# spartan-array/spartan

Measured on AMD Instinct MI355X. Metric: spartan.dot TFLOP/s (+ map/reduce HBM GB/s), higher is better.
Workload: dtype f32

## Files before the change

### spartan_amd/csrc/gemm_split.hpp

```cpp
#pragma once

typedef __bf16 gs_bf16x8 __attribute__((ext_vector_type(8)));
typedef __bf16 gs_bf16x4 __attribute__((ext_vector_type(4)));

namespace {

constexpr int GS_BK = 16;
constexpr int GS_RB = GS_BK * 2;
constexpr int GS_WN = 4;
constexpr unsigned GS_WIN_LO = (127u - 40u) << 23;
constexpr unsigned GS_WIN_HI = (127u + 40u) << 23;
constexpr size_t GS_IMAGE_CAP = (size_t)2 << 30;
constexpr size_t GS_WS_HEAD = 512;

template <int WN>
struct GsCfg {
  static constexpr int BM = 256, BN = 64 * WN, NW = 2 * WN, THREADS = 64 * NW;
  static constexpr int A_BYTES = BM * GS_RB, B_BYTES = BN * GS_RB;
  static constexpr int STAGE_BYTES = 3 * A_BYTES + 3 * B_BYTES;
  static constexpr int SMEM_BYTES = 2 * STAGE_BYTES;
  static constexpr int APW = A_BYTES / 1024 / NW, BPW = B_BYTES / 1024 / NW;
  static constexpr int NPIECES = 3 * APW + 3 * BPW;
  static constexpr int SLOTS = SP_CUS * (WN == 4 ? 1 : 2);
  static_assert(APW >= 1 && BPW >= 1 && APW * NW * 1024 == A_BYTES && BPW * NW * 1024 == B_BYTES, "tile / waves mismatch");
  static_assert(NPIECES * 4 <= 48, "one piece after every fourth MFMA");
};

__device__ __forceinline__ bool gs_outside(float v) {
  const unsigned b = __float_as_uint(v) & 0x7fffffffu;
  return b != 0u && (b < GS_WIN_LO || b >= GS_WIN_HI);
}

__device__ __forceinline__ void gs_cut(float v, __bf16& h, __bf16& m, __bf16& l) {
  h = (__bf16)v;
  const float r1 = v - (float)h;
  m = (__bf16)r1;
  l = (__bf16)(r1 - (float)m);
}

__device__ __forceinline__ void gs_raise(bool bad, unsigned* flag) {
  if (__any(bad) && (threadIdx.x & 63) == 0) atomicOr(flag, 1u);
}

__global__ __launch_bounds__(256) void sp_gemm_cut_rows_kernel(const float* __restrict__ A, int64_t lda, int M, int K,
                                                               __bf16* __restrict__ Ah, int64_t img,
                                                               unsigned* __restrict__ flag) {
  const int q = threadIdx.x & 7, row = blockIdx.x * 32 + (threadIdx.x >> 3);
  const int kpad = (K + GS_BK - 1) / GS_BK * GS_BK;
  bool bad = false;
  if (row < M) {
    const float* __restrict__ a = A + (int64_t)row * lda;
#pragma unroll
    for (int it = 0; it < 8; ++it) {
      const int k = blockIdx.y * 256 + it * 32 + 4 * q;
      if (k >= kpad) break;
      f32x4 v = {0.f, 0.f, 0.f, 0.f};
      if (k + 4 <= K) {
        v = *(const f32x4*)(a + k);
      } else {
#pragma unroll
        for (int e = 0; e < 4; ++e)
          if (k + e < K) v[e] = a[k + e];
      }
      gs_bf16x4 h, m, l;
#pragma unroll
      for (int e = 0; e < 4; ++e) {
        bad |= gs_outside(v[e]);
        __bf16 hh, mm, ll;
        gs_cut(v[e], hh, mm, ll);
        h[e] = hh;
        m[e] = mm;
        l[e] = ll;
      }
      const int64_t at = ((int64_t)(k >> 4) * M + row) * GS_BK + (k & 15);
      *(gs_bf16x4*)(Ah + at) = h;
      *(gs_bf16x4*)(Ah + img + at) = m;
      *(gs_bf16x4*)(Ah + 2 * img + at) = l;
    }
  }
  gs_raise(bad, flag);
}

__global__ __launch_bounds__(256) void sp_gemm_cut_cols_kernel(const float* __restrict__ B, int64_t ldb, int N, int K,
                                                               __bf16* __restrict__ Bh, int64_t img,
                                                               unsigned* __restrict__ flag) {
  __shared__ __attribute__((aligned(16))) __bf16 s[3][256 * GS_BK];
  const int n0 = blockIdx.x * 256, col = n0 + threadIdx.x, k0 = blockIdx.y * GS_BK;
  float v[GS_BK];
#pragma unroll
  for (int e = 0; e < GS_BK; ++e) v[e] = (col < N && k0 + e < K) ? B[(int64_t)(k0 + e) * ldb + col] : 0.f;
  bool bad = false;
  gs_bf16x8 h[2], m[2], l[2];
#pragma unroll
  for (int e = 0; e < GS_BK; ++e) {
    bad |= gs_outside(v[e]);
    __bf16 hh, mm, ll;
    gs_cut(v[e], hh, mm, ll);
    h[e >> 3][e & 7] = hh;
    m[e >> 3][e & 7] = mm;
    l[e >> 3][e & 7] = ll;
  }
#pragma unroll
  for (int c = 0; c < 2; ++c) {
    *(gs_bf16x8*)(&s[0][threadIdx.x * GS_BK + 8 * c]) = h[c];
    *(gs_bf16x8*)(&s[1][threadIdx.x * GS_BK + 8 * c]) = m[c];
    *(gs_bf16x8*)(&s[2][threadIdx.x * GS_BK + 8 * c]) = l[c];
  }
  __syncthreads();
  const int64_t base = ((int64_t)blockIdx.y * N + n0) * GS_BK;
#pragma unroll
  for (int p = 0; p < 3; ++p)
#pragma unroll
    for (int c = 0; c < 2; ++c) {
      const int at = (c * 256 + threadIdx.x) * 8;
      if (n0 + at / GS_BK < N) *(gs_bf16x8*)(Bh + p * img + base + at) = *(const gs_bf16x8*)(&s[p][at]);
    }
  gs_raise(bad, flag);
}

template <int WN>
__global__ __launch_bounds__(GsCfg<WN>::THREADS, 2) void sp_gemm_glds_kernel_bf16x3(
    const char* __restrict__ Ah, int64_t a_img, const char* __restrict__ Bh, int64_t b_img, float* __restrict__ C,
    int64_t ldc, int M, int N, int KT, int accumulate, int tiles_m, int tiles_n, const unsigned* __restrict__ flag) {
  using G = GsCfg<WN>;
  constexpr int APW = G::APW, BPW = G::BPW, NPIECES = G::NPIECES;
  extern __shared__ __attribute__((aligned(16))) char gs_smem[];
  if (*flag != 0u) return;
  int tm, tn;
  sp_gemm_tile_of_block(blockIdx.x, gridDim.x, tiles_m, tiles_n, tm, tn);
  const int m0 = tm * G::BM, n0 = tn * G::BN;
  const int tid = threadIdx.x, lane = tid & 63;
  const int wid = __builtin_amdgcn_readfirstlane(tid >> 6);
  const int wm = wid / WN, wn = wid % WN;
  const int l31 = lane & 31, lh = lane >> 5;

  unsigned a_off[APW], b_off[BPW];
#pragma unroll
  for (int j = 0; j < APW; ++j) {
    const int slot = (wid * APW + j) * 64 + lane;
    int row = slot >> 1;
    const int q = (slot & 1) ^ ((row >> 4) & 1);
    if (m0 + row > M - 1) row = M - 1 - m0;
    a_off[j] = (unsigned)(row * GS_RB + q * 16);
  }
#pragma unroll
  for (int j = 0; j < BPW; ++j) {
    const int slot = (wid * BPW + j) * 64 + lane;
    int row = slot >> 1;
    const int q = (slot & 1) ^ ((row >> 4) & 1);
    if (n0 + row > N - 1) row = N - 1 - n0;
    b_off[j] = (unsigned)(row * GS_RB + q * 16);
  }
  const char* __restrict__ Ablk = Ah + (int64_t)m0 * GS_RB;
  const char* __restrict__ Bblk = Bh + (int64_t)n0 * GS_RB;
  const int64_t a_slab = (int64_t)M * GS_RB, b_slab = (int64_t)N * GS_RB;
  const unsigned s_base = SP_LDS_ADDR(gs_smem);

#define GS_PIECE(i)                                                                                    \
  do {                                                                                                 \
    if ((i) < 3 * APW) {                                                                               \
      const int p_ = (i) / APW, j_ = (i) % APW;                                                        \
      SP_GLDS_S(Ablk + p_ * a_img + ka_, a_off[j_], st_ + p_ * G::A_BYTES + (wid * APW + j_) * 1024);  \
    } else {                                                                                           \
      const int p_ = ((i) - 3 * APW) / BPW, j_ = ((i) - 3 * APW) % BPW;                                \
      SP_GLDS_S(Bblk + p_ * b_img + kb_, b_off[j_],                                                    \
                st_ + 3 * G::A_BYTES + p_ * G::B_BYTES + (wid * BPW + j_) * 1024);                     \
    }                                                                                                  \
  } while (0)

  f32x16 acc[4][2];
#pragma unroll
  for (int i = 0; i < 4; ++i)
#pragma unroll
    for (int j = 0; j < 2; ++j)
#pragma unroll
      for (int r = 0; r < 16; ++r) acc[i][j][r] = 0.f;

  {
    const int64_t ka_ = 0, kb_ = 0;
    const unsigned st_ = s_base;
#pragma unroll
    for (int i = 0; i < NPIECES; ++i) GS_PIECE(i);
  }
  SP_GLDS_LANDED();
  __syncthreads();

  const int fslot = (lh ^ ((l31 >> 4) & 1)) * 16;
  const int a_frag = (wm * 128 + l31) * GS_RB + fslot;
  const int b_frag = 3 * G::A_BYTES + (wn * 64 + l31) * GS_RB + fslot;

  for (int t = 0; t < KT; ++t) {
    const bool more = t + 1 < KT;
    const int64_t ka_ = (int64_t)(t + 1) * a_slab, kb_ = (int64_t)(t + 1) * b_slab;
    const unsigned st_ = s_base + (unsigned)((t + 1) & 1) * G::STAGE_BYTES;
    const char* st = gs_smem + (t & 1) * G::STAGE_BYTES;
    gs_bf16x8 af[3][4], bf[3][2];
#pragma unroll
    for (int p = 0; p < 3; ++p) {
#pragma unroll
      for (int i = 0; i < 4; ++i) af[p][i] = *(const gs_bf16x8*)(st + p * G::A_BYTES + a_frag + i * 32 * GS_RB);
#pragma unroll
      for (int j = 0; j < 2; ++j) bf[p][j] = *(const gs_bf16x8*)(st + p * G::B_BYTES + b_frag + j * 32 * GS_RB);
    }
    int piece = 0;
#pragma unroll
    for (int idx = 0; idx < 48; ++idx) {
      const int term = idx >> 3, i = (idx & 7) >> 1, j = idx & 1;
      const int pa = term == 0 ? 2 : (term == 2 || term == 3) ? 1 : 0;
      const int pb = term == 1 ? 2 : (term == 2 || term == 4) ? 1 : 0;
      acc[i][j] = __builtin_amdgcn_mfma_f32_32x32x16_bf16(af[pa][i], bf[pb][j], acc[i][j], 0, 0, 0);
      if (idx % 4 == 3 && piece < NPIECES) {
        __builtin_amdgcn_sched_barrier(0);
        if (more) GS_PIECE(piece);
        __builtin_amdgcn_sched_barrier(0);
        ++piece;
      }
    }
    if (more) SP_GLDS_LANDED();
    __syncthreads();
  }
#undef GS_PIECE

#pragma unroll
  for (int i = 0; i < 4; ++i) {
#pragma unroll
    for (int j = 0; j < 2; ++j) {
      const int col = n0 + wn * 64 + j * 32 + l31;
#pragma unroll
      for (int r = 0; r < 16; ++r) {
        const int row = m0 + wm * 128 + i * 32 + (r & 3) + 8 * (r >> 2) + 4 * lh;
        if (row < M && col < N) {
          float* p = C + (int64_t)row * ldc + col;
          float v = acc[i][j][r];
          if (accumulate) v += *p;
          *p = v;
        }
      }
    }
  }
}

template <typename Cfg, int BM, int BN, int WM, int WN, int WGS>
__global__ __launch_bounds__(Cfg::THREADS, WGS) void sp_gemm_f32_gated_kernel(
    const float* __restrict__ A, int64_t lda, const float* __restrict__ B, int64_t ldb, float* __restrict__ C,
    int64_t ldc, int M, int N, int K, int accumulate, int tiles_m, int tiles_n, const unsigned* __restrict__ flag) {
  if (*flag == 0u) return;
  sp_gemm_glds_body<Cfg, BM, BN, WM, WN>(A, lda, B, ldb, C, ldc, M, N, K, accumulate, tiles_m, tiles_n);
}

#define GS_CUT_BYTES_PER_S 3.0e12
#define GS_ISSUED_FLOPS 1.1e15
static bool sp_gemm_bf16_plan(int64_t M, int64_t N, int64_t K) {
  static int mode = -2;
  if (mode == -2) {
    const char* e = getenv("SP_GEMM_SPLIT");
    mode = e ? atoi(e) : 1;
  }
  using G = GsCfg<GS_WN>;
  if (mode == 0 || K < 16 || N % 4 != 0 || N < 4 || M < 1 || M > 2147483647LL || N > 2147483647LL || K > 2147483647LL)
    return false;
  const int64_t tb = ((M + 255) / 256) * ((N + 127) / 128);
  if (tb < 2 * SP_CUS || tb >= 2147483647LL) return false;
  double dp_cost;
  if (sp_gemm_dp_choice(M, N, &dp_cost) != 6 || sp_sk_plan(M, N, K)) return false;
  const int64_t KT = (K + GS_BK - 1) / GS_BK;
  if ((double)KT * 3.0 * GS_RB * ((double)M + (double)N) > (double)GS_IMAGE_CAP) return false;
  const double fp32_s = dp_cost * 128.0 * 128.0 * (double)K * 2.0 / (157.3e12 * 0.95 / SP_CUS);
  const int64_t tiles = ((M + G::BM - 1) / G::BM) * ((N + G::BN - 1) / G::BN);
  const int64_t rounds = (tiles + G::SLOTS - 1) / G::SLOTS;
  const double main_s = (double)rounds * G::SLOTS * (6.0 * 2.0 * G::BM * G::BN * (double)K) / GS_ISSUED_FLOPS;
  const double cut_s = 10.0 * ((double)M + (double)N) * (double)K / GS_CUT_BYTES_PER_S;
  return (main_s + cut_s + 20e-6) < 0.92 * fp32_s;
}

static size_t sp_gemm_bf16_ws_bytes(int64_t M, int64_t N, int64_t K) {
  return GS_WS_HEAD + (size_t)((K + GS_BK - 1) / GS_BK) * 3 * GS_RB * (size_t)(M + N);
}

static int sp_gemm_bf16_launch(const float* A, int64_t lda, const float* B, int64_t ldb, float* C, int64_t ldc, int64_t M,
                               int64_t N, int64_t K, int acc, void* ws, hipStream_t st) {
  using G = GsCfg<GS_WN>;
  char* base = (char*)(((uintptr_t)ws + 255) & ~(uintptr_t)255);
  unsigned* flag = (unsigned*)base;
  const int64_t KT = (K + GS_BK - 1) / GS_BK;
  const int64_t a_img = KT * M * GS_RB, b_img = KT * N * GS_RB;
  char* Aimg = base + 256;
  char* Bimg = Aimg + 3 * a_img;
  const int64_t tiles_m = (M + G::BM - 1) / G::BM, tiles_n = (N + G::BN - 1) / G::BN;
  auto kern = sp_gemm_glds_kernel_bf16x3<GS_WN>;
  using FCfg = GldsCfg<256, 128, 2, 2>;
  auto gated = sp_gemm_f32_gated_kernel<FCfg, 256, 128, 2, 2, 2>;
  static bool attr_set = false;
  if (!attr_set) {
    SP_HIP(hipFuncSetAttribute((const void*)kern, hipFuncAttributeMaxDynamicSharedMemorySize, G::SMEM_BYTES));
    SP_HIP(hipFuncSetAttribute((const void*)gated, hipFuncAttributeMaxDynamicSharedMemorySize, FCfg::LDS_BYTES));
    attr_set = true;
  }
  SP_HIP(hipMemsetAsync(flag, 0, 256, st));
  hipLaunchKernelGGL(sp_gemm_cut_rows_kernel, dim3((unsigned)((M + 31) / 32), (unsigned)((K + 255) / 256)), dim3(256), 0, st,
                     A, lda, (int)M, (int)K, (__bf16*)Aimg, a_img / 2, flag);
  hipLaunchKernelGGL(sp_gemm_cut_cols_kernel, dim3((unsigned)((N + 255) / 256), (unsigned)KT), dim3(256), 0, st, B, ldb,
                     (int)N, (int)K, (__bf16*)Bimg, b_img / 2, flag);
  hipLaunchKernelGGL(kern, dim3((unsigned)(tiles_m * tiles_n)), dim3(G::THREADS), G::SMEM_BYTES, st, (const char*)Aimg,
                     a_img, (const char*)Bimg, b_img, C, ldc, (int)M, (int)N, (int)KT, acc, (int)tiles_m, (int)tiles_n,
                     (const unsigned*)flag);
  const int64_t ftm = (M + 255) / 256, ftn = (N + 127) / 128;
  hipLaunchKernelGGL(gated, dim3((unsigned)(ftm * ftn)), dim3(FCfg::THREADS), FCfg::LDS_BYTES, st, A, lda, B, ldb, C, ldc,
                     (int)M, (int)N, (int)K, acc, (int)ftm, (int)ftn, (const unsigned*)flag);
  SP_CHECK_LAUNCH();
  return 0;
}

}
```

### spartan_amd/csrc/sp_common.hpp

```cpp
#pragma once
#include <hip/hip_runtime.h>
#include <stdint.h>
#ifndef __HIPCC_RTC__
#include <stdio.h>
#include <string.h>
#endif

#include "../../include/spartan_hip.h"

void sp_set_error(const char* fmt, ...);

#define SP_FAIL(...)          \
  do {                        \
    sp_set_error(__VA_ARGS__); \
    return 1;                 \
  } while (0)

#define SP_HIP(expr)                                                              \
  do {                                                                            \
    hipError_t e_ = (expr);                                                       \
    if (e_ != hipSuccess) {                                                       \
      sp_set_error("%s:%d: %s failed: %s", __FILE__, __LINE__, #expr,             \
                   hipGetErrorString(e_));                                        \
      return 1;                                                                   \
    }                                                                             \
  } while (0)

#define SP_CHECK_LAUNCH()                                                         \
  do {                                                                            \
    hipError_t e_ = hipGetLastError();                                            \
    if (e_ != hipSuccess) {                                                       \
      sp_set_error("%s:%d: kernel launch failed: %s", __FILE__, __LINE__,         \
                   hipGetErrorString(e_));                                        \
      return 1;                                                                   \
    }                                                                             \
  } while (0)

__host__ __device__ static inline size_t sp_dtype_size(int32_t dt) {
  switch (dt) {
    case SP_F32: return 4;
    case SP_F64: return 8;
    case SP_I32: return 4;
    case SP_I64: return 8;
    case SP_BOOL: return 1;
    case SP_U8: return 1;
    case SP_I8: return 1;
    case SP_I16: return 2;
    case SP_U16: return 2;
    case SP_U32: return 4;
    case SP_F16: return 2;
    default: return 0;
  }
}

#define SP_CUS 256
#define SP_BLOCKS_PER_CU 8
#define SP_BLOCK 256

#ifndef __HIPCC_RTC__
#define SP_GLDS_LANDED() asm volatile("s_waitcnt vmcnt(0)" ::: "memory")
#define SP_GLDS_S(base, voff, lds_addr)                                                             \
  asm volatile("s_mov_b32 m0, %0\n\ts_nop 0\n\tglobal_load_lds_dwordx4 %1, %2"                       \
               :: "s"(lds_addr), "v"(voff), "s"(base) : "memory")
#define SP_GLDS_V(gptr, lds_addr)                                                                   \
  asm volatile("s_mov_b32 m0, %0\n\ts_nop 0\n\tglobal_load_lds_dwordx4 %1, off"                      \
               :: "s"(lds_addr), "v"(gptr) : "memory")
#define SP_LDS_ADDR(p) ((unsigned)(uintptr_t)(__attribute__((address_space(3))) void*)(p))
#endif

struct sp_inputs {
  const void* p[SP_MAX_INPUTS];
};
```

Before: 249.9.

## Triple-buffer split-bf16 GEMM LDS ring and widen row-cut kernel to 8 elements

The split-bf16 GEMM main loop moves from a two-stage to a three-stage LDS ring. It prefetches two k-tiles ahead and waits with a partial vmcnt count, so the tile for the next iteration can land while the one after it is still in flight. The row-cut preprocessing kernel now handles 8 floats per thread per iteration and stores 16-byte bf16x8 vectors instead of 8-byte ones. The fragment loads are also reordered to fetch the term pairs in MFMA consumption order. The larger LDS footprint may lower blocks per CU for the smaller WN configuration.

```diff
diff --git a/spartan_amd/csrc/gemm_split.hpp b/spartan_amd/csrc/gemm_split.hpp
--- a/spartan_amd/csrc/gemm_split.hpp
+++ b/spartan_amd/csrc/gemm_split.hpp
@@ -18,12 +18,14 @@
   static constexpr int BM = 256, BN = 64 * WN, NW = 2 * WN, THREADS = 64 * NW;
   static constexpr int A_BYTES = BM * GS_RB, B_BYTES = BN * GS_RB;
   static constexpr int STAGE_BYTES = 3 * A_BYTES + 3 * B_BYTES;
-  static constexpr int SMEM_BYTES = 2 * STAGE_BYTES;
+  static constexpr int STAGES = 3;
+  static constexpr int SMEM_BYTES = STAGES * STAGE_BYTES;
   static constexpr int APW = A_BYTES / 1024 / NW, BPW = B_BYTES / 1024 / NW;
   static constexpr int NPIECES = 3 * APW + 3 * BPW;
   static constexpr int SLOTS = SP_CUS * (WN == 4 ? 1 : 2);
   static_assert(APW >= 1 && BPW >= 1 && APW * NW * 1024 == A_BYTES && BPW * NW * 1024 == B_BYTES, "tile / waves mismatch");
   static_assert(NPIECES * 4 <= 48, "one piece after every fourth MFMA");
+  static_assert(NPIECES <= 31 && SMEM_BYTES <= 160 * 1024, "two k-tiles of requests in vmcnt; the ring in a CU's LDS");
 };
 
 __device__ __forceinline__ bool gs_outside(float v) {
@@ -51,31 +53,33 @@
   if (row < M) {
     const float* __restrict__ a = A + (int64_t)row * lda;
 #pragma unroll
-    for (int it = 0; it < 8; ++it) {
-      const int k = blockIdx.y * 256 + it * 32 + 4 * q;
+    for (int it = 0; it < 4; ++it) {
+      const int k = blockIdx.y * 256 + it * 64 + 8 * q;
       if (k >= kpad) break;
-      f32x4 v = {0.f, 0.f, 0.f, 0.f};
-      if (k + 4 <= K) {
-        v = *(const f32x4*)(a + k);
+      f32x4 v[2] = {{0.f, 0.f, 0.f, 0.f}, {0.f, 0.f, 0.f, 0.f}};
+      if (k + 8 <= K) {
+        v[0] = *(const f32x4*)(a + k);
+        v[1] = *(const f32x4*)(a + k + 4);
       } else {
 #pragma unroll
-        for (int e = 0; e < 4; ++e)
-          if (k + e < K) v[e] = a[k + e];
+        for (int e = 0; e < 8; ++e)
+          if (k + e < K) v[e >> 2][e & 3] = a[k + e];
       }
-      gs_bf16x4 h, m, l;
-#pragma unroll
-      for (int e = 0; e < 4; ++e) {
-        bad |= gs_outside(v[e]);
+      gs_bf16x8 h, m, l;
+#pragma unroll
+      for (int e = 0; e < 8; ++e) {
+        const float x = v[e >> 2][e & 3];
+        bad |= gs_outside(x);
         __bf16 hh, mm, ll;
-        gs_cut(v[e], hh, mm, ll);
+        gs_cut(x, hh, mm, ll);
         h[e] = hh;
         m[e] = mm;
         l[e] = ll;
       }
       const int64_t at = ((int64_t)(k >> 4) * M + row) * GS_BK + (k & 15);
-      *(gs_bf16x4*)(Ah + at) = h;
-      *(gs_bf16x4*)(Ah + img + at) = m;
-      *(gs_bf16x4*)(Ah + 2 * img + at) = l;
+      *(gs_bf16x8*)(Ah + at) = h;
+      *(gs_bf16x8*)(Ah + img + at) = m;
+      *(gs_bf16x8*)(Ah + 2 * img + at) = l;
     }
   }
   gs_raise(bad, flag);
@@ -182,25 +186,36 @@
 #pragma unroll
     for (int i = 0; i < NPIECES; ++i) GS_PIECE(i);
   }
-  SP_GLDS_LANDED();
+  if (KT > 1) {
+    const int64_t ka_ = a_slab, kb_ = b_slab;
+    const unsigned st_ = s_base + G::STAGE_BYTES;
+#pragma unroll
+    for (int i = 0; i < NPIECES; ++i) GS_PIECE(i);
+    SP_GLDS_LANDED_BUT(NPIECES);
+  } else {
+    SP_GLDS_LANDED();
+  }
   __syncthreads();
 
   const int fslot = (lh ^ ((l31 >> 4) & 1)) * 16;
   const int a_frag = (wm * 128 + l31) * GS_RB + fslot;
   const int b_frag = 3 * G::A_BYTES + (wn * 64 + l31) * GS_RB + fslot;
 
+  int cur = 0;
   for (int t = 0; t < KT; ++t) {
-    const bool more = t + 1 < KT;
-    const int64_t ka_ = (int64_t)(t + 1) * a_slab, kb_ = (int64_t)(t + 1) * b_slab;
-    const unsigned st_ = s_base + (unsigned)((t + 1) & 1) * G::STAGE_BYTES;
-    const char* st = gs_smem + (t & 1) * G::STAGE_BYTES;
+    const bool more = t + 2 < KT;
+    const int nxt = cur == 0 ? 2 : cur - 1;
+    const int64_t ka_ = (int64_t)(t + 2) * a_slab, kb_ = (int64_t)(t + 2) * b_slab;
+    const unsigned st_ = s_base + (unsigned)nxt * G::STAGE_BYTES;
+    const char* st = gs_smem + cur * G::STAGE_BYTES;
     gs_bf16x8 af[3][4], bf[3][2];
 #pragma unroll
-    for (int p = 0; p < 3; ++p) {
-#pragma unroll
-      for (int i = 0; i < 4; ++i) af[p][i] = *(const gs_bf16x8*)(st + p * G::A_BYTES + a_frag + i * 32 * GS_RB);
-#pragma unroll
-      for (int j = 0; j < 2; ++j) bf[p][j] = *(const gs_bf16x8*)(st + p * G::B_BYTES + b_frag + j * 32 * GS_RB);
+    for (int g = 0; g < 3; ++g) {
+      const int pa = g == 0 ? 2 : g == 1 ? 0 : 1, pb = g == 0 ? 0 : g == 1 ? 2 : 1;
+#pragma unroll
+      for (int i = 0; i < 4; ++i) af[pa][i] = *(const gs_bf16x8*)(st + pa * G::A_BYTES + a_frag + i * 32 * GS_RB);
+#pragma unroll
+      for (int j = 0; j < 2; ++j) bf[pb][j] = *(const gs_bf16x8*)(st + pb * G::B_BYTES + b_frag + j * 32 * GS_RB);
     }
     int piece = 0;
 #pragma unroll
@@ -216,8 +231,10 @@
         ++piece;
       }
     }
-    if (more) SP_GLDS_LANDED();
+    if (more) SP_GLDS_LANDED_BUT(NPIECES);
+    else SP_GLDS_LANDED();
     __syncthreads();
+    cur = cur == 2 ? 0 : cur + 1;
   }
 #undef GS_PIECE
 
diff --git a/spartan_amd/csrc/sp_common.hpp b/spartan_amd/csrc/sp_common.hpp
--- a/spartan_amd/csrc/sp_common.hpp
+++ b/spartan_amd/csrc/sp_common.hpp
@@ -59,6 +59,7 @@
 
 #ifndef __HIPCC_RTC__
 #define SP_GLDS_LANDED() asm volatile("s_waitcnt vmcnt(0)" ::: "memory")
+#define SP_GLDS_LANDED_BUT(n) asm volatile("s_waitcnt vmcnt(%0)" :: "n"(n) : "memory")
 #define SP_GLDS_S(base, voff, lds_addr)                                                             \
   asm volatile("s_mov_b32 m0, %0\n\ts_nop 0\n\tglobal_load_lds_dwordx4 %1, %2"                       \
                :: "s"(lds_addr), "v"(voff), "s"(base) : "memory")
```

New measurement: 244.6. 0.979x the previous value.
